# gaozhihan/PreDiff

Measured on AMD Instinct MI355X. Metric: denoising_steps_per_sec, higher is better.
Workload: dtype bf16; 1 GPU; SEVIR-LR 7->6 x128x128 (latent 13x16x16, C 256/512, depth [4,4], axial), DDIM-50 eta=0, no knowledge alignment (BASELINE.json configs[1]); trajectories_per_gpu=64, global_trajectories=64, sampler=ddim50, hip_graph=True, lanes=2, trajectories_per_launch=32, parallelism=ensemble-shard x1

## Files before the change

prediff_amd/csrc/conv3d_halo.hip:

```cpp
#include <algorithm>
#include "common.h"
#include "igemm_epilogue.h"

namespace PD_NS {

#define BLDS16(rsrc, ldsptr, voff, soff) \
  __builtin_amdgcn_raw_ptr_buffer_load_lds((rsrc), (__attribute__((address_space(3))) void*)(ldsptr), 16, (voff), (soff), 0, 0)
#define PD_OOB 0xffffff00u
#define VMCNT(n) asm volatile("s_waitcnt vmcnt(" #n ")" ::: "memory")
#define PHASE_SYNC()                   \
  __builtin_amdgcn_sched_barrier(0);   \
  __builtin_amdgcn_s_barrier();        \
  __builtin_amdgcn_sched_barrier(0)

namespace {
constexpr int FW = 16;
constexpr int HW = FW + 2;
constexpr int HROWS = HW * HW;
constexpr int PLROWS = 336;
constexpr int PLANE = PLROWS * 16;
constexpr int HALO = 8 * PLANE;
constexpr int NPIECE = HALO / 1024;
constexpr int WHT = 128 * 128;
constexpr int WBUF = 2 * WHT;
static_assert(PLANE % 256 == 0 && HALO % 1024 == 0 && PLROWS >= HROWS, "halo plane layout");
constexpr int FW1 = 8;
constexpr int RP1 = 9;
constexpr int FR1 = 81;
constexpr int FPAIR1 = 88;
constexpr int WROW1 = 169;
constexpr int FREACH1 = 91;
constexpr int PLROWS1 = 352;
static_assert(FPAIR1 % 16 == 8 && FPAIR1 >= FR1 && WROW1 + FPAIR1 + FREACH1 <= PLROWS1, "level-1 halo plane layout");
constexpr int frame_base1(int f) { return (f >> 1) * WROW1 + (f & 1) * FPAIR1; }

template <int L>
struct Lay {
  static constexpr int ROWS = L ? PLROWS1 : PLROWS;
  static constexpr int PLANE = ROWS * 16;
  static constexpr int HALO = 8 * PLANE;
  static constexpr int NPIECE = HALO / 1024;
  static constexpr int NEXTRA = NPIECE - 40;
  static constexpr int PITCH = L ? RP1 : HW;
  static constexpr int W_OFF = 2 * HALO;
  static constexpr int LDS = W_OFF + 2 * WBUF;
  static_assert(PLANE % 256 == 0 && HALO % 1024 == 0 && NEXTRA >= 0 && NEXTRA <= 8, "halo plane layout");
  static_assert(LDS >= 8 * 128 * 32 * 4 && LDS <= 160 * 1024, "the epilogue stages 128 KB of accumulators in the operand buffers; a CU has 160 KB");
};

struct FragH {
  op8 v[2];
};
}

template <int L, bool BORDER>
__global__ void __launch_bounds__(512) conv3d_halo_kernel(const pd_igemm_args p) {
#if defined(__HIP_DEVICE_COMPILE__)
  constexpr int PLROWS = Lay<L>::ROWS, PLANE = Lay<L>::PLANE, HALO = Lay<L>::HALO, NEXTRA = Lay<L>::NEXTRA, PITCH = Lay<L>::PITCH,
                W_OFF = Lay<L>::W_OFF;
  extern __shared__ __attribute__((aligned(16))) char smem[];
  const int tid = threadIdx.x;
  const int lane = tid & 63;
  const int wave = __builtin_amdgcn_readfirstlane(tid >> 6);
  const int wr = wave >> 2, wc = wave & 3;

  const int tiles_n = (p.N + 255) >> 8;
  const int tiles_m = L ? (p.M + 255) >> 8 : p.M >> 8;
  const int nt = tiles_m * tiles_n;
  int t;
  {
    const int bid = blockIdx.x, xcd = bid & 7, q = nt >> 3, r = nt & 7;
    t = (xcd < r ? xcd * (q + 1) : r * (q + 1) + (xcd - r) * q) + (bid >> 3);
  }
  const int tm = t / tiles_n;
  const int m0 = tm << 8;
  const int n0 = (t % tiles_n) << 8;

  const auto rA = __builtin_amdgcn_make_buffer_rsrc((void*)p.A, 0, p.a_bytes, 0x00020000);
  const auto rW = __builtin_amdgcn_make_buffer_rsrc((void*)p.W, 0, p.w_bytes, 0x00020000);

  const int srow = tid >> 3, spos = tid & 7;
  const uint32_t w_sel = (uint32_t)(spos ^ ((srow >> 1) & 7)) * 16u;
  uint32_t woff[2][2];
#pragma unroll
  for (int hh = 0; hh < 2; ++hh)
#pragma unroll
    for (int i = 0; i < 2; ++i) {
      const int n = n0 + hh * 128 + i * 64 + srow;
      woff[hh][i] = n < p.N ? ((uint32_t)n * (uint32_t)p.ldw) * 2u + w_sel : PD_OOB;
    }
  uint32_t hoff[6];
#pragma unroll
  for (int n = 0; n < 6; ++n) {
    const int cell = (wave + 8 * n) * 64 + lane;
    const int s = cell / PLROWS, r = cell - s * PLROWS;
    if constexpr (L == 0) {
      const int hr = r / HW, hc = r - hr * HW;
      const bool ok = cell < 8 * PLROWS && r < HROWS && hr >= 1 && hr <= FW && hc >= 1 && hc <= FW;
      hoff[n] = ok ? (uint32_t)((hr - 1) * FW + (hc - 1)) * (uint32_t)p.lda * 2u + (uint32_t)s * 16u : PD_OOB;
    } else {
      hoff[n] = PD_OOB | 4u;
#pragma unroll
      for (int f = 0; f < 4; ++f) {
        const int rel = r - frame_base1(f), hr = rel / RP1, hc = rel - hr * RP1;
        if (cell < 8 * PLROWS && rel >= 0 && rel < FR1 && hr >= 1 && hc >= 1)
          hoff[n] = ((uint32_t)(f * (FW1 * FW1) + (hr - 1) * FW1 + (hc - 1)) * (uint32_t)p.lda * 2u + (uint32_t)s * 16u) | (uint32_t)f;
      }
    }
  }

  const int kchunks = p.Cin >> 6;
  const int ot = tm % p.To;
  const bool dense = (p.debug_flags & 8) != 0;
  const int kt_lo = (dense || L) ? 0 : max(0, 1 - ot), kt_hi = (dense || L) ? 2 : min(2, p.Ti - ot);
  const int ngroups = (p.debug_flags & 1) ? 0 : kchunks * (kt_hi - kt_lo + 1);
  const uint32_t frame_b = (uint32_t)(L ? FW1 * FW1 : FW * FW) * (uint32_t)p.lda * 2u;
  uint32_t vm_all = 0;
  if constexpr (L == 1) {
    int o = (4 * tm) % p.To;
    for (int f = 0; f < 4; ++f) {
      if (4 * tm + f < p.B * p.To)
        for (int kt = 0; kt < 3; ++kt)
          if ((unsigned)(o - 1 + kt) < (unsigned)p.Ti) vm_all |= 1u << (4 * kt + f);
      if (++o == p.To) o = 0;
    }
  }
  const uint32_t w_tap_b = (uint32_t)p.w_tap_stride * 2u;

  int h_c = 0, h_kt = kt_lo, w_c = 0, w_kt = kt_lo;
  uint32_t w_off = (uint32_t)(kt_lo * 9) * w_tap_b;
  int h_soff = 0;
  uint32_t h_mask = 0, h_back = 0;
  char* const h_dst = smem + wave * 1024;
  char* const w_dst = smem + W_OFF + wave * 1024;
  auto next_halo = [&]() {
    if constexpr (L == 0) {
      const int it = ot - 1 + h_kt;
      const bool ok = (unsigned)it < (unsigned)p.Ti;
      h_soff = __builtin_amdgcn_readfirstlane(ok ? (int)((uint32_t)(tm - 1 + h_kt) * frame_b + (uint32_t)h_c * 128u) : 0);
      h_mask = ok ? 0u : PD_OOB;
    } else {
      const int fin = 4 * tm - 1 + h_kt, fb = max(fin, 0);
      h_soff = __builtin_amdgcn_readfirstlane((int)((uint32_t)fb * frame_b + (uint32_t)h_c * 128u));
      h_back = (uint32_t)(fb - fin) * frame_b;
      h_mask = (vm_all >> (4 * h_kt)) & 15u;
    }
    if (++h_kt > kt_hi) { h_kt = kt_lo; ++h_c; }
  };
  auto issue_h = [&](int n, int buf) {
    uint32_t v;
    if constexpr (L == 0) v = hoff[n] | h_mask;
    else v = ((h_mask >> (hoff[n] & 7u)) & 1u) ? (hoff[n] & ~7u) - h_back : PD_OOB;
    BLDS16(rA, h_dst + buf * HALO + n * 8192, v, h_soff);
  };
  auto next_w_group = [&]() {
    if (++w_kt > kt_hi) { w_kt = kt_lo; ++w_c; }
    w_off = (uint32_t)(w_kt * 9) * w_tap_b + (uint32_t)w_c * 128u;
  };
  auto issue_w = [&](int buf) {
    const int so = __builtin_amdgcn_readfirstlane((int)w_off);
    char* dst = w_dst + buf * WBUF;
    BLDS16(rW, dst, woff[0][0], so);
    BLDS16(rW, dst + 64 * 128, woff[0][1], so);
    BLDS16(rW, dst + WHT, woff[1][0], so);
    BLDS16(rW, dst + WHT + 64 * 128, woff[1][1], so);
    w_off += w_tap_b;
  };

  f32x4 acc[8][4];
#pragma unroll
  for (int i = 0; i < 8; ++i)
#pragma unroll
    for (int j = 0; j < 4; ++j)
#pragma unroll
      for (int r = 0; r < 4; ++r) acc[i][j][r] = 0.f;

  const int l16 = lane & 15, lg = lane >> 4;
  const int swz = (l16 >> 1) & 7;
  const int a_rd = (L ? wr * WROW1 + (l16 >> 3) * FPAIR1 + (l16 & 7) : wr * (8 * HW) + l16) * 16 + lg * PLANE;
  const int b_rd = W_OFF + (wc >> 1) * WHT + ((wc & 1) * 64 + l16) * 128;

  if (ngroups > 0) {
    next_halo();
    if (wave < NEXTRA) issue_h(5, 0);
#pragma unroll
    for (int n = 0; n < 5; ++n) issue_h(n, 0);
    issue_w(0);
    issue_w(1);
    VMCNT(4);
  }
  __builtin_amdgcn_s_barrier();
  if (wr == 1) __builtin_amdgcn_s_barrier();
  __builtin_amdgcn_sched_barrier(0);

  FragH a[4], b0[2], b1[2];
#define LOAD_B(f, base) \
  (f).v[0] = *(const op8*)((base) + ((lg ^ swz) * 16)); (f).v[1] = *(const op8*)((base) + (((4 + lg) ^ swz) * 16))
#define LOAD_A(f, base) \
  (f).v[0] = *(const op8*)(base); (f).v[1] = *(const op8*)((base) + 4 * PLANE)
#define QUAD16(R0, C0, bfrag, SK)                                                                           \
  _Pragma("unroll") for (int ks = 0; ks < 2; ++ks)                                                          \
    _Pragma("unroll") for (int i = 0; i < 4; ++i)                                                           \
      if (i != (SK))                                                                                        \
        _Pragma("unroll") for (int c = 0; c < 2; ++c)                                                       \
          acc[(R0) + i][(C0) + c] = mfma_16x16x32(a[i].v[ks], bfrag[c].v[ks], acc[(R0) + i][(C0) + c]);

  int wcur = 0;
  auto group = [&](auto has_next_t, auto wr_t, int g) {
    constexpr bool has_next = decltype(has_next_t)::value;
    constexpr int WR = decltype(wr_t)::value;
    constexpr bool skip_top = BORDER && (L == 1 || WR == 0), skip_bot = BORDER && (L == 1 || WR == 1);
    const int hnxt = (g & 1) ^ 1;
    const char* sA = smem + (g & 1) * HALO + a_rd;
    if (has_next) next_halo();
#pragma unroll
    for (int j = 0; j < 9; ++j) {
      const int shift = ((j / 3) * PITCH + (j % 3)) * 16;
      const char* sB = smem + wcur * WBUF + b_rd;
      const int skA = j < 3 && skip_top ? 0 : -1, skB = j >= 6 && skip_bot ? 3 : -1;
#pragma unroll
      for (int c = 0; c < 2; ++c) { LOAD_B(b0[c], sB + c * (16 * 128)); }
#pragma unroll
      for (int i = 0; i < 4; ++i)
        if (i != skA) { LOAD_A(a[i], sA + shift + i * (PITCH * 16)); }
#pragma unroll
      for (int c = 0; c < 2; ++c) { LOAD_B(b1[c], sB + (2 + c) * (16 * 128)); }
      if (j >= 1 && j <= 5 && has_next) {
        if (j == 1 && wave < NEXTRA) issue_h(5, hnxt);
        issue_h(j - 1, hnxt);
      }
      PHASE_SYNC();
      __builtin_amdgcn_s_setprio(1);
      QUAD16(0, 0, b0, skA)
      QUAD16(0, 2, b1, skA)
      __builtin_amdgcn_s_setprio(0);
      PHASE_SYNC();
#pragma unroll
      for (int i = 0; i < 4; ++i)
        if (i != skB) { LOAD_A(a[i], sA + shift + (4 + i) * (PITCH * 16)); }
      if (j <= 6 || has_next) {
        if (j == 7) next_w_group();
        issue_w(wcur);
        if (j >= 1 && j <= 5 && has_next) {
          VMCNT(5);
        } else {
          VMCNT(4);
        }
      } else {
        VMCNT(0);
      }
      PHASE_SYNC();
      __builtin_amdgcn_s_setprio(1);
      QUAD16(4, 2, b1, skB)
      QUAD16(4, 0, b0, skB)
      __builtin_amdgcn_s_setprio(0);
      PHASE_SYNC();
      wcur ^= 1;
    }
  };
  auto groups = [&](auto wr_t) {
    for (int g = 0; g + 1 < ngroups; ++g) group(std::true_type{}, wr_t, g);
    if (ngroups > 0) group(std::false_type{}, wr_t, ngroups - 1);
  };
  if constexpr (L == 0 && BORDER) {
    if (wr == 0) groups(std::integral_constant<int, 0>{});
    else groups(std::integral_constant<int, 1>{});
  } else {
    groups(std::integral_constant<int, -1>{});
  }
#undef QUAD16
#undef LOAD_A
#undef LOAD_B
  if (wr == 0) __builtin_amdgcn_s_barrier();
  if (p.debug_flags & 2) return;

  float* sC = (float*)smem + wave * (128 * 32);
  const int m_base = m0 + wr * 128;
  const int m_end = min(p.M, m_base + 128);
  const int c_row = L ? (lg >> 1) * 64 + (lg & 1) * 4 : 4 * lg;
  auto slab = [&](auto jsc) {
    constexpr int js = decltype(jsc)::value;
    if (js == 0) __syncthreads();
    else igemm_epilogue_wave_sync();
#pragma unroll
    for (int i = 0; i < 8; ++i)
#pragma unroll
      for (int c = 0; c < 2; ++c)
#pragma unroll
        for (int r = 0; r < 4; ++r) sC[(c_row + i * (L ? 8 : 16) + r) * 32 + c * 16 + l16] = acc[i][js * 2 + c][r];
    igemm_epilogue_wave_sync();
    igemm_epilogue<128, 32>(p, sC, lane, m_base, m_end, n0 + wc * 64 + js * 32, 0);
  };
  slab(std::integral_constant<int, 0>{});
  slab(std::integral_constant<int, 1>{});
#endif
}

bool pd_conv3d_halo_supported(const pd_igemm_args& a, int kind, int level) {
  if (kind != 2 || a.split || a.fp8 || a.w_fold > 0 || a.nbatch > 1) return false;
  if (a.KT != 3 || a.KH != 3 || a.KW != 3 || a.pt != 1 || a.ph != 1 || a.pw != 1) return false;
  if (a.st != 1 || a.sh != 1 || a.sw != 1 || a.ut != 1 || a.uh != 1 || a.uw != 1 || a.vT > 0 || a.vH > 0 || a.vW > 0) return false;
  const int fw = level ? FW1 : FW;
  return a.Hi == fw && a.Wi == fw && a.Ho == fw && a.Wo == fw && a.Ti == a.To;
}

template <int L, bool BORDER>
static int launch_halo(const pd_igemm_args& a, hipStream_t s) {
  constexpr int LDS = Lay<L>::LDS;
  static bool attr_set_dev[PD_MAX_DEVICES];
  if (int rc = pd_raise_lds("pd_igemm", (const void*)conv3d_halo_kernel<L, BORDER>, LDS, attr_set_dev)) return rc;
  const int tiles = ((a.M + 255) / 256) * ((a.N + 255) / 256);
  hipLaunchKernelGGL((conv3d_halo_kernel<L, BORDER>), dim3(tiles, 1, 1), dim3(512), LDS, s, a);
  PD_CHECK_LAUNCH();
  return PD_OK;
}

int pd_conv3d_halo_launch(const pd_igemm_args& a, int level, hipStream_t s) {
  if (a.debug_flags & 256) return level ? launch_halo<1, false>(a, s) : launch_halo<0, false>(a, s);
  return level ? launch_halo<1, true>(a, s) : launch_halo<0, true>(a, s);
}

}
```

Baseline: 1733 steps/s.

## Add sample-aligned level-1 halo conv tiles that skip out-of-range temporal taps

For level-1 3D convs, when the batch is a multiple of four, each 256-row tile now holds the same output frame from four different samples instead of four consecutive frames. Every frame in a tile then shares one temporal boundary condition, so the kernel can use the uniform kt_lo/kt_hi range and skip whole k-groups for the border frames, as level 0 already does, rather than loading masked halos for all three taps. The epilogue writes two 64-row slices per wave to scattered output rows. This adds a third template instantiation and a new path that debug flag 512 can switch off.

```diff
diff --git a/prediff_amd/csrc/conv3d_halo.hip b/prediff_amd/csrc/conv3d_halo.hip
--- a/prediff_amd/csrc/conv3d_halo.hip
+++ b/prediff_amd/csrc/conv3d_halo.hip
@@ -53,8 +53,9 @@
 };
 }
 
-template <int L, bool BORDER>
+template <int L, bool BORDER, bool ALIGNED = false>
 __global__ void __launch_bounds__(512) conv3d_halo_kernel(const pd_igemm_args p) {
+  static_assert(!ALIGNED || L == 1, "the sample-aligned frame slots are a level-1 form: a level-0 tile is one frame");
 #if defined(__HIP_DEVICE_COMPILE__)
   constexpr int PLROWS = Lay<L>::ROWS, PLANE = Lay<L>::PLANE, HALO = Lay<L>::HALO, NEXTRA = Lay<L>::NEXTRA, PITCH = Lay<L>::PITCH,
                 W_OFF = Lay<L>::W_OFF;
@@ -65,7 +66,7 @@
   const int wr = wave >> 2, wc = wave & 3;
 
   const int tiles_n = (p.N + 255) >> 8;
-  const int tiles_m = L ? (p.M + 255) >> 8 : p.M >> 8;
+  const int tiles_m = ALIGNED ? (p.B >> 2) * p.To : L ? (p.M + 255) >> 8 : p.M >> 8;
   const int nt = tiles_m * tiles_n;
   int t;
   {
@@ -98,6 +99,14 @@
       const int hr = r / HW, hc = r - hr * HW;
       const bool ok = cell < 8 * PLROWS && r < HROWS && hr >= 1 && hr <= FW && hc >= 1 && hc <= FW;
       hoff[n] = ok ? (uint32_t)((hr - 1) * FW + (hc - 1)) * (uint32_t)p.lda * 2u + (uint32_t)s * 16u : PD_OOB;
+    } else if constexpr (ALIGNED) {
+      hoff[n] = PD_OOB;
+#pragma unroll
+      for (int f = 0; f < 4; ++f) {
+        const int rel = r - frame_base1(f), hr = rel / RP1, hc = rel - hr * RP1;
+        if (cell < 8 * PLROWS && rel >= 0 && rel < FR1 && hr >= 1 && hc >= 1)
+          hoff[n] = (uint32_t)(f * p.Ti * (FW1 * FW1) + (hr - 1) * FW1 + (hc - 1)) * (uint32_t)p.lda * 2u + (uint32_t)s * 16u;
+      }
     } else {
       hoff[n] = PD_OOB | 4u;
 #pragma unroll
@@ -112,11 +121,12 @@
   const int kchunks = p.Cin >> 6;
   const int ot = tm % p.To;
   const bool dense = (p.debug_flags & 8) != 0;
-  const int kt_lo = (dense || L) ? 0 : max(0, 1 - ot), kt_hi = (dense || L) ? 2 : min(2, p.Ti - ot);
+  constexpr bool UNIFORM = L == 0 || ALIGNED;
+  const int kt_lo = (dense || !UNIFORM) ? 0 : max(0, 1 - ot), kt_hi = (dense || !UNIFORM) ? 2 : min(2, p.Ti - ot);
   const int ngroups = (p.debug_flags & 1) ? 0 : kchunks * (kt_hi - kt_lo + 1);
   const uint32_t frame_b = (uint32_t)(L ? FW1 * FW1 : FW * FW) * (uint32_t)p.lda * 2u;
   uint32_t vm_all = 0;
-  if constexpr (L == 1) {
+  if constexpr (L == 1 && !ALIGNED) {
     int o = (4 * tm) % p.To;
     for (int f = 0; f < 4; ++f) {
       if (4 * tm + f < p.B * p.To)
@@ -134,10 +144,11 @@
   char* const h_dst = smem + wave * 1024;
   char* const w_dst = smem + W_OFF + wave * 1024;
   auto next_halo = [&]() {
-    if constexpr (L == 0) {
+    if constexpr (UNIFORM) {
       const int it = ot - 1 + h_kt;
       const bool ok = (unsigned)it < (unsigned)p.Ti;
-      h_soff = __builtin_amdgcn_readfirstlane(ok ? (int)((uint32_t)(tm - 1 + h_kt) * frame_b + (uint32_t)h_c * 128u) : 0);
+      const int fin = ALIGNED ? 4 * (tm / p.To) * p.Ti + it : tm - 1 + h_kt;
+      h_soff = __builtin_amdgcn_readfirstlane(ok ? (int)((uint32_t)fin * frame_b + (uint32_t)h_c * 128u) : 0);
       h_mask = ok ? 0u : PD_OOB;
     } else {
       const int fin = 4 * tm - 1 + h_kt, fb = max(fin, 0);
@@ -149,7 +160,7 @@
   };
   auto issue_h = [&](int n, int buf) {
     uint32_t v;
-    if constexpr (L == 0) v = hoff[n] | h_mask;
+    if constexpr (UNIFORM) v = hoff[n] | h_mask;
     else v = ((h_mask >> (hoff[n] & 7u)) & 1u) ? (hoff[n] & ~7u) - h_back : PD_OOB;
     BLDS16(rA, h_dst + buf * HALO + n * 8192, v, h_soff);
   };
@@ -289,7 +300,16 @@
 #pragma unroll
         for (int r = 0; r < 4; ++r) sC[(c_row + i * (L ? 8 : 16) + r) * 32 + c * 16 + l16] = acc[i][js * 2 + c][r];
     igemm_epilogue_wave_sync();
-    igemm_epilogue<128, 32>(p, sC, lane, m_base, m_end, n0 + wc * 64 + js * 32, 0);
+    if constexpr (ALIGNED) {
+      const int row0 = ((4 * (tm / p.To) + 2 * wr) * p.To + ot) * (FW1 * FW1);
+#pragma unroll 1
+      for (int h = 0; h < 2; ++h) {
+        const int mb = row0 + h * p.To * (FW1 * FW1);
+        igemm_epilogue<64, 32>(p, sC + h * (64 * 32), lane, mb, mb + 64, n0 + wc * 64 + js * 32, 0);
+      }
+    } else {
+      igemm_epilogue<128, 32>(p, sC, lane, m_base, m_end, n0 + wc * 64 + js * 32, 0);
+    }
   };
   slab(std::integral_constant<int, 0>{});
   slab(std::integral_constant<int, 1>{});
@@ -304,20 +324,23 @@
   return a.Hi == fw && a.Wi == fw && a.Ho == fw && a.Wo == fw && a.Ti == a.To;
 }
 
-template <int L, bool BORDER>
+template <int L, bool BORDER, bool ALIGNED = false>
 static int launch_halo(const pd_igemm_args& a, hipStream_t s) {
   constexpr int LDS = Lay<L>::LDS;
   static bool attr_set_dev[PD_MAX_DEVICES];
-  if (int rc = pd_raise_lds("pd_igemm", (const void*)conv3d_halo_kernel<L, BORDER>, LDS, attr_set_dev)) return rc;
+  if (int rc = pd_raise_lds("pd_igemm", (const void*)conv3d_halo_kernel<L, BORDER, ALIGNED>, LDS, attr_set_dev)) return rc;
   const int tiles = ((a.M + 255) / 256) * ((a.N + 255) / 256);
-  hipLaunchKernelGGL((conv3d_halo_kernel<L, BORDER>), dim3(tiles, 1, 1), dim3(512), LDS, s, a);
+  hipLaunchKernelGGL((conv3d_halo_kernel<L, BORDER, ALIGNED>), dim3(tiles, 1, 1), dim3(512), LDS, s, a);
   PD_CHECK_LAUNCH();
   return PD_OK;
 }
 
 int pd_conv3d_halo_launch(const pd_igemm_args& a, int level, hipStream_t s) {
-  if (a.debug_flags & 256) return level ? launch_halo<1, false>(a, s) : launch_halo<0, false>(a, s);
-  return level ? launch_halo<1, true>(a, s) : launch_halo<0, true>(a, s);
-}
-
-}
+  const bool border = !(a.debug_flags & 256);
+  if (!level) return border ? launch_halo<0, true>(a, s) : launch_halo<0, false>(a, s);
+  if (a.B % 4 == 0 && a.M == a.B * a.To * (FW1 * FW1) && !(a.debug_flags & 512))
+    return border ? launch_halo<1, true, true>(a, s) : launch_halo<1, false, true>(a, s);
+  return border ? launch_halo<1, true>(a, s) : launch_halo<1, false>(a, s);
+}
+
+}
```

Result: no change. 1748 steps/s, median of 6 (+0.9%).
